# BosonHBC/BHRayTracer

Measured on AMD Instinct MI355X. Metric: Mrays/s (closest-hit + any-hit rays per second), with wall-clock per frame, higher is better.
Workload: dtype f32

## Files before the change

bhraytracer_amd/csrc/device_state.h:

```cpp
#pragma once

namespace bhrt {

template <class T> struct DevBuf {
    T *p = nullptr;
    size_t n = 0;
    DevBuf() = default;
    DevBuf(const DevBuf &) = delete;
    DevBuf &operator=(const DevBuf &) = delete;
    DevBuf(DevBuf &&o) noexcept : p(o.p), n(o.n) { o.p = nullptr; o.n = 0; }
    DevBuf &operator=(DevBuf &&o) noexcept
    {
        if (this != &o) { Free(); p = o.p; n = o.n; o.p = nullptr; o.n = 0; }
        return *this;
    }
    ~DevBuf() { Free(); }
    int Reserve(size_t want)
    {
        if (n >= want) return BHRT_OK;
        Free();
        HIP_CHECK(hipMalloc(&p, want * sizeof(T)));
        n = want;
        return BHRT_OK;
    }
// ... 115 lines not shown
    DevBuf<float> d_slowf;
    DevBuf<uint32_t> d_slowu;
    DevBuf<float> d_shf2;
    DevBuf<uint32_t> d_shu2;
    DevBuf<uint32_t> d_order_sh;
    DevBuf<uint32_t> d_seg_sh;
    DevBuf<Counters> d_cnt_sh;
    DevBuf<Counters> d_cnt;
    PinnedBuf<HostCounters> h_pub;
    HostCounters *d_pub = nullptr;
    uint32_t pub_seq = 0;
    int timers = 0;
    struct PendingTimer { int e0, e1; double *acc; };
    std::vector<PendingTimer> ev_pending;
    std::vector<int> ev_free;
    DevBuf<DPhoton> d_photons;
    uint32_t n_photons = 0;
    std::vector<HostPhoton> h_photons;
    DevBuf<float> d_ph_frames;
    DevBuf<float4> d_ph_hot, d_ph_cold, d_ph_dbox;
    PhotonMapDev pm;
    GatherWorkspace gw;
    struct Knobs {
        int stream_waves = -1;
        bool fused_camera = true;
        bool no_slow_queue = false;
        bool debug_slow = false, debug_gather = false, debug_drain = false;
        bool balance_host = false;
        int frame_cap = 0;
        int gather_lane_budget = 0;
        bool gather_counting_sort = false;
        bool shadow_overlap = true;
        bool fused_resolve = true;
        int gather_stats = 0;
        void FromEnv()
        {
            if (const char *e = getenv("BHRT_STREAM_WAVES")) stream_waves = atoi(e);
            if (const char *e = getenv("BHRT_FUSED_CAMERA")) fused_camera = atoi(e) != 0;
            no_slow_queue = getenv("BHRT_NO_SLOW_QUEUE") != nullptr;
            debug_slow = getenv("BHRT_DEBUG_SLOW") != nullptr; debug_gather = getenv("BHRT_DEBUG_GATHER") != nullptr; debug_drain = getenv("BHRT_DEBUG_DRAIN") != nullptr;
            if (const char *e = getenv("BHRT_PHOTON_BALANCE_HOST")) balance_host = atoi(e) != 0;
            if (const char *e = getenv("BHRT_GATHER_COUNTING_SORT")) gather_counting_sort = atoi(e) != 0;
            if (const char *e = getenv("BHRT_SHADOW_OVERLAP")) shadow_overlap = atoi(e) != 0;
            if (const char *e = getenv("BHRT_FUSED_RESOLVE")) fused_resolve = atoi(e) != 0;
        }
    } knobs;
    uint64_t pass_hint_key = 0;
    uint32_t pass_hint = 0;
    uint64_t frames_seen_key = 0;
    double frames_seen = 0;
    size_t frame_px = 0;
    DevBuf<uint8_t> d_frame_rgb;
    DevBuf<float> d_frame_rad, d_frame_var;
    DevBuf<uint32_t> d_frame_cnt;
    DevBuf<uint8_t> d_ad;
    DevBuf<uint8_t> d_dn;
    size_t api_cap = 0;
    DevBuf<float> d_api_f;
    DevBuf<int32_t> d_api_i;
};

void DestroyDeviceState(DeviceState *d)
{
    if (!d) return;
    if (d->device >= 0) (void)hipSetDevice(d->device);
    delete d;
}

}
```

bhraytracer_amd/csrc/kernels.hip:

```cpp
#include <hip/hip_runtime.h>

#include <stdlib.h>
#include <string.h>

#include <algorithm>
#include <type_traits>
#include <chrono>
#include <string>
#include <vector>

#include "bhrt.h"
#include "denoise.h"
#include "device_color24.h"
#include "device_photon.h"
#include "photon_host.h"
#include "scene_internal.h"

namespace bhrt {

#define HIP_CHECK(expr)                                                                                        \
    do {                                                                                                       \
        hipError_t e_ = (expr);                                                                                \
        if (e_ != hipSuccess) {                                                                                \
            SetError(std::string(#expr) + ": " + hipGetErrorString(e_));                                       \
// ... 184 lines not shown
{
    const uint32_t lane = __lane_id();
    const uint64_t lt = (1ull << lane) - 1ull;
    const uint64_t m0 = __ballot(cls == RC_HEAVY), m1 = __ballot(cls == RC_MEDIUM), m2 = __ballot(cls == RC_LIGHT), m3 = __ballot(cls == RC_MESH);
    uint32_t base = 0;
    if (lane < 4) {
        const uint64_t mk = lane == 0 ? m0 : (lane == 1 ? m1 : (lane == 2 ? m2 : m3));
        const uint32_t c = (uint32_t)__popcll(mk);
        if (c) base = atomicAdd(&cnt->cls[lane][shard].v, c);
    }
    const uint32_t wshard = shard;
    const uint32_t b0 = __shfl(base, 0), b1 = __shfl(base, 1), b2 = __shfl(base, 2), b3 = __shfl(base, 3);
    if (cls != RC_NONE) {
        const uint64_t mm = cls == RC_HEAVY ? m0 : (cls == RC_MEDIUM ? m1 : (cls == RC_LIGHT ? m2 : m3));
        const uint32_t pos = (cls == RC_HEAVY ? b0 : (cls == RC_MEDIUM ? b1 : (cls == RC_LIGHT ? b2 : b3))) + (uint32_t)__popcll(mm & lt);
        if (pos < ord.shard_cap) ord.idx[((size_t)cls * BHRT_ORDER_SHARDS + wshard) * ord.shard_cap + pos] = i;
        else atomicOr(&cnt->overflow.v, 8u);
    }
}
__device__ inline uint32_t shading_class(uint32_t meta, const Hit &hit)
{
    const uint32_t kind = meta & 15u;
    const bool is_hit = hit.node >= 0;
    bool heavy = false;
    if (is_hit) {
        if (kind == RK_CAMERA) heavy = true;
        else if (kind == RK_GI) heavy = fabsf(hit.t) > BHRT_BIAS;
        else if (kind == RK_REFR_IN) heavy = hit.front != 0;
        else heavy = true;
    }
    return heavy ? RC_HEAVY : ((kind == RK_REFR_IN && is_hit) ? RC_MEDIUM : RC_LIGHT);
}

struct SlowQueue {
    RayQueue q;
    uint32_t cap;
};
constexpr uint32_t kSlowCap = 1u << 16;
template <bool kPark, bool kCamera, bool kMeshes = true>
__global__ void __launch_bounds__(kBlock) k_trace_closest(DevScene S, PassInfo P, RayQueue q, uint32_t n, int uniform_side, HitBuf h, RayOrder ord, Counters *cnt,
                                                          SlowQueue slow )
{
    __shared__ bhrt_bvh_node nodelet[(kPark || !kMeshes) ? 1 : BHRT_LDS_NODES];
    const uint32_t i = blockIdx.x * blockDim.x + threadIdx.x;
    bool active = i < n;
    V3 o = v3(0, 0, 0), d = v3(0, 0, 1);
    uint32_t meta = 0;
    if (active) fetch_ray<kCamera>(S, P, q, i, o, d, meta);
    const bool has_meta = kCamera || q.meta;
    const int side = has_meta ? (int)((meta >> 4) & 3u) : uniform_side;
    const bool dead = has_meta && (meta & 15u) == RK_DEAD;
    Hit hit;
    uint32_t key = 0;
    bool is_slow = false;
    int parked = trace_closest<kMeshes>(S, o, d, side, hit, active && !dead, (kPark || !kMeshes) ? nullptr : nodelet, 0, kPark, kPark ? &key : nullptr,
                                        (uint16_t *)nullptr, 0, BHRT_LDS_NODES, kCamera, kPark ? &is_slow : nullptr);
    if (kPark && parked >= 0 && is_slow && slow.cap) {
        const uint32_t k = atomicAdd(&cnt->n_slow.v, 1u);
        if (k < slow.cap) {
            slow.q.ox[k] = o.x; slow.q.oy[k] = o.y; slow.q.oz[k] = o.z; slow.q.dx[k] = d.x; slow.q.dy[k] = d.y; slow.q.dz[k] = d.z;
            slow.q.frame[k] = kCamera ? i : q.frame[i];
            slow.q.meta[k] = meta;
            slow.q.rng_ctr[k] = (kCamera || (meta & 15u) == RK_GI) ? 0u : q.rng_ctr[i];
            active = false;
            parked = -1;
        }
    }
    if (active) { h.t[i] = hit.t; h.node[i] = hit.node; h.prim[i] = hit.prim; h.front[i] = hit.front | ((parked + 1) << 8); }
    if (kPark && parked >= 0) {
        ord.park_key[i] = key;
        if (!kCamera) ord.park_rank[i] = atomicAdd(&ord.park_bucket[key], 1u);
    }
    if (!ord.idx) return;
    uint32_t cls = RC_NONE;
    if (active && !dead) cls = parked >= 0 ? (uint32_t)RC_MESH : shading_class(meta, hit);
    file_ray(cls, i, (i >> 10) & (BHRT_ORDER_SHARDS - 1) , ord, cnt);
}
__device__ inline bool parked_entry(const RayOrder &ord, uint32_t b, uint32_t *s_seg, uint32_t &i, uint32_t first_entry = 0 )
{
    __syncthreads();
    if (threadIdx.x < 64) {
        const uint32_t l = threadIdx.x;
        const uint32_t a = l <= BHRT_ORDER_SHARDS ? ord.mesh_start[l] : 0xffffffffu;
        const uint32_t n_le = (uint32_t)__popcll(__ballot(l < BHRT_ORDER_SHARDS && a <= b));
        if (l == 0) *s_seg = n_le - 1;
    }
    __syncthreads();
    if (b >= ord.mesh_start[BHRT_ORDER_SHARDS]) return false;
    const uint32_t seg = *s_seg;
    const uint32_t local = (b - ord.mesh_start[seg]) * kBlock + first_entry + threadIdx.x;
    const bool active = local < ord.mesh_count[seg];
    i = active ? ord.idx[((size_t)RC_MESH * BHRT_ORDER_SHARDS + seg) * ord.shard_cap + local] : 0xffffffffu;
    return true;
}
#ifndef BHRT_XCD_LOCAL
#define BHRT_XCD_LOCAL 0
#endif
__device__ inline bool xcd_slice(uint32_t b, uint32_t nb, uint32_t &slice)
{
    slice = b;
#if BHRT_XCD_LOCAL
    constexpr uint32_t G = BHRT_XCD_LOCAL, span = 8 * G;
    const uint32_t chunk = b / span, in = b % span;
    if ((chunk + 1) * span <= nb) slice = chunk * span + (in & 7u) * G + (in >> 3);
#endif
    return b < nb;
}
__global__ void __launch_bounds__(kBlock) k_park_scatter(RayOrder ord)
{
    __shared__ uint32_t s_seg;
    uint32_t i;
    for (uint32_t b = blockIdx.x; parked_entry(ord, b, &s_seg, i); b += gridDim.x)
        if (i != 0xffffffffu) ord.park_sorted[ord.park_bucket[ord.park_key[i]] + ord.park_rank[i]] = i;
}
constexpr uint32_t kMeshNodelet = 256;
#ifndef BHRT_MESH_BLOCK
#define BHRT_MESH_BLOCK 64
#endif
constexpr int kMeshBlock = BHRT_MESH_BLOCK;
template <bool kCamera, int kPath, bool kLS = false>
__global__ void __launch_bounds__(kCamera ? kBlock : kMeshBlock, kPath == 1 ? 6 : 4 ) k_trace_mesh(DevScene S, PassInfo P, RayQueue q, HitBuf h, RayOrder ord, Counters *cnt)
{
    typedef typename std::conditional<kPath == 2, uint32_t, uint16_t>::type PathT;
    constexpr int kTB = kCamera ? kBlock : kMeshBlock;
    __shared__ bhrt_bvh_node nodelet[kPath ? 1 : kMeshNodelet];
    __shared__ PathT path[kPath ? 33 * kTB : 1];
    __shared__ uint32_t s_seg;
    bool active;
    uint32_t i;
    uint32_t slice;
    if (kCamera) {
        if (!xcd_slice(blockIdx.x, ord.mesh_start[BHRT_ORDER_SHARDS], slice)) return;
        if (!parked_entry(ord, slice, &s_seg, i)) return;
        active = i != 0xffffffffu;
        if (!active) i = 0;
    } else {
        const uint32_t total = ord.mesh_count[BHRT_ORDER_SHARDS];
        if (!xcd_slice(blockIdx.x, (total + kTB - 1) / kTB, slice)) return;
        const uint32_t k = slice * kTB + threadIdx.x;
        active = k < total;
        i = active ? ord.park_sorted[k] : 0u;
    }
    V3 o = v3(0, 0, 0), d = v3(0, 0, 1);
    uint32_t meta = 0;
    Hit hit = {BHRT_BIGFLOAT, -1, -1, 1};
    int start = 0;
    if (active) {
        fetch_ray<kCamera>(S, P, q, i, o, d, meta);
        hit.t = h.t[i]; hit.node = h.node[i]; hit.prim = h.prim[i];
        const int fw = h.front[i];
        hit.front = fw & 0xff;
        start = (fw >> 8) - 1;
    }
    trace_closest<true, PathT, kLS>(S, o, d, (int)((meta >> 4) & 3u), hit, active, kPath ? nullptr : nodelet, active ? start : S.n_nodes, false, nullptr,
                               kPath ? path + threadIdx.x : (PathT *)nullptr, kTB, kMeshNodelet);
    if (active) { h.t[i] = hit.t; h.node[i] = hit.node; h.prim[i] = hit.prim; h.front[i] = hit.front; }
    if (kCamera) file_ray(active ? shading_class(meta, hit) : (uint32_t)RC_NONE, i, slice & (BHRT_ORDER_SHARDS - 1), ord, cnt);
}
#ifndef BHRT_STREAM_REFILL
#define BHRT_STREAM_REFILL 32
#endif
constexpr int kStreamRefill = BHRT_STREAM_REFILL;
#ifndef BHRT_STREAM_OCC
#define BHRT_STREAM_OCC 6
#endif
#ifdef BHRT_DEBUG_DRAIN
__device__ unsigned long long g_stream_t[4];
#endif
#ifdef BHRT_DEBUG_STREAM
__device__ unsigned long long g_stream_dbg[8];
#endif
template <int kPath, bool kLS = false>
__global__ void __launch_bounds__(64, kPath == 1 ? BHRT_STREAM_OCC : (BHRT_STREAM_OCC < 5 ? BHRT_STREAM_OCC : 5) ) k_trace_mesh_stream(DevScene S, RayQueue q, HitBuf h, RayOrder ord, Counters *cnt)
{
    typedef typename std::conditional<kPath == 2, uint32_t, uint16_t>::type PathT;
    __shared__ PathT path[33 * 64];
    const uint32_t total = ord.mesh_count[BHRT_ORDER_SHARDS];
    const uint32_t lane = threadIdx.x;
    PathT *stack = path + lane;
    bool have = false, pending = false, exhausted = false;
    uint32_t i = 0;
    int n = 0, side = 0;
    Hit hit = {BHRT_BIGFLOAT, -1, -1, 1};
    MeshWalk W = {};
    W.st = 3;
    int cur_n = -1;
    MeshRef M = mesh_ref(S, 0);
#ifdef BHRT_DEBUG_STREAM
    unsigned long long dbg[8] = {0, 0, 0, 0, 0, 0, 0, 0};
    unsigned long long c_mark = __builtin_readcyclecounter();
// ... 69 lines not shown
#endif
        for (;;) {
            const int nD = __popcll(__ballot(W.st == 0)), nL = __popcll(__ballot(W.st == 1)), nC = __popcll(__ballot(W.st == 2));
            const int walking = nD + nL + nC;
            if (walking == 0 || (!exhausted && 64 - walking - n_wait >= kStreamRefill)) break;
#ifdef BHRT_DEBUG_STREAM
#if BHRT_FUSED_CLIMB
            dbg[0]++; dbg[1] += walking; dbg[2] += (nD >= nL && nD > 0) ? nD : nL;
            if (nD >= nL && nD > 0) dbg[6]++; else if (nL > 0) dbg[7]++;
#else
            dbg[0]++; dbg[1] += walking; dbg[2] += (nD >= nL && nD >= nC) ? nD : (nL >= nC ? nL : nC);
            if (nD >= nL && nD >= nC) dbg[6]++; else if (nL >= nC) dbg[7]++;
#endif
#endif
#ifdef BHRT_DEBUG_STREAM
            const unsigned long long r0 = __builtin_readcyclecounter();
#endif
            walk_round<PathT, kLS>(M, W, side, hit.t, hit.prim, hit.front, stack, 64u, nD, nL, nC);
#ifdef BHRT_DEBUG_STREAM
            if (nD >= nL && nD > 0) dbg[4] += __builtin_readcyclecounter() - r0;
#endif
        }
#ifdef BHRT_DEBUG_STREAM
        { const unsigned long long c = __builtin_readcyclecounter(); dbg[3] += c - c_mark; c_mark = c; }
#endif
    }
#ifdef BHRT_DEBUG_STREAM
    if (lane == 0) for (int k = 0; k < 8; k++) atomicAdd(&g_stream_dbg[k], dbg[k]);
#endif
#ifdef BHRT_DEBUG_DRAIN
    if (lane == 0) atomicMax(&g_stream_t[2], wall_clock64());
#endif
}
__global__ void __launch_bounds__(kBlock) k_file_parked(RayQueue q, HitBuf h, RayOrder ord, Counters *cnt)
{
    __shared__ uint32_t s_seg;
    uint32_t i;
    if (!parked_entry(ord, blockIdx.x, &s_seg, i)) return;
    const bool active = i != 0xffffffffu;
    uint32_t cls = RC_NONE;
    if (active) {
        Hit hit;
        hit.t = h.t[i]; hit.node = h.node[i]; hit.prim = h.prim[i]; hit.front = h.front[i];
        cls = shading_class(q.meta[i], hit);
    }
    file_ray(cls, active ? i : 0u, blockIdx.x & (BHRT_ORDER_SHARDS - 1), ord, cnt);
}

__global__ void __launch_bounds__(64) k_trace_slow(DevScene S, SlowQueue slow, uint32_t a, uint32_t b, HitBuf h)
{
    __shared__ CoopLds lds;
    __builtin_amdgcn_s_setprio(3);
    const uint32_t i = a + blockIdx.x;
    if (i >= b) return;
    const V3 o = v3(slow.q.ox[i], slow.q.oy[i], slow.q.oz[i]), d = v3(slow.q.dx[i], slow.q.dy[i], slow.q.dz[i]);
    const uint32_t meta = slow.q.meta[i];
    Hit hit;
#ifdef BHRT_DEBUG_LONG_RAYS
    const unsigned long long c0 = wall_clock64();
#endif
    trace_closest_coop(S, lds, o, d, (int)((meta >> 4) & 3u), hit);
#ifdef BHRT_DEBUG_LONG_RAYS
    const double ms = (double)(wall_clock64() - c0) / 1e5;
    if (threadIdx.x == 0 && ms > 5.0) printf("slow ray %u: %.1f ms o=(%.9g %.9g %.9g) d=(%.9g %.9g %.9g) side %u -> node %d prim %d t %.9g\n", i, ms, o.x, o.y, o.z, d.x, d.y, d.z, (meta >> 4) & 3u, hit.node, hit.prim, hit.t);
#endif
    if (threadIdx.x == 0) { h.t[i] = hit.t; h.node[i] = hit.node; h.prim[i] = hit.prim; h.front[i] = hit.front; }
}
__global__ void __launch_bounds__(kBlock) k_inject_slow(RayQueue sq, HitBuf sh, uint32_t src0, uint32_t m, RayQueue q, HitBuf h, uint32_t dst0)
{
    const uint32_t k = blockIdx.x * blockDim.x + threadIdx.x;
    if (k >= m) return;
    const uint32_t a = src0 + k, b = dst0 + k;
    q.ox[b] = sq.ox[a]; q.oy[b] = sq.oy[a]; q.oz[b] = sq.oz[a]; q.dx[b] = sq.dx[a]; q.dy[b] = sq.dy[a]; q.dz[b] = sq.dz[a];
    q.frame[b] = sq.frame[a]; q.meta[b] = sq.meta[a]; q.rng_ctr[b] = sq.rng_ctr[a];
    h.t[b] = sh.t[a]; h.node[b] = sh.node[a]; h.prim[b] = sh.prim[a]; h.front[b] = sh.front[a];
}
static inline uint32_t kFileAllBlocks(uint32_t first, uint32_t n) { return (n - (first & ~63u) + kBlock - 1) / kBlock; }
// ... 363 lines not shown
                code = pcode * 2;
                how = FH_REFR_FRONT;
            } else {
                code = pcode * 2;
                how = FH_REFR_OUT;
                const bhrt_material &pm = S.materials[(F.info[owner] >> 20) & 0xfffu];
                V3 af = v3(dm::powf_(BHRT_EULER, -pm.absorption[0] * hit.t), dm::powf_(BHRT_EULER, -pm.absorption[1] * hit.t),
                           dm::powf_(BHRT_EULER, -pm.absorption[2] * hit.t));
                mult = ld3i(F.refr_color, owner) * af;
            }
        }
        F.parent[f] = owner;
        F.info2[f] = (uint32_t)(gi + 64) | ((uint32_t)(bounce & 0xff) << 8);
        F.skey[f] = skey;
        F.code[f] = code;
        if (how == FH_REFR_OUT) st3(F.mult, f, mult);
        const int mi = kFm ? resolve_material(S, F.fm, hit.node, hit.prim) : S.nodes[hit.node].material;
        bool need_uv = kTex && mi >= 0 && (S.materials[mi].diffuse.map >= 0 || S.materials[mi].specular.map >= 0);
        if (kLe && mi >= 0) need_uv = need_uv || F.emission[mi].map >= 0;
        Attr a;
        hit_attrs(S, o, d, hit.t, hit.node, hit.prim, need_uv, a);
        shade_entry<kTex, kLe, kFm>(S, R, F, f, how, o, a, hit.node, mi, bounce, gi, code, skey, so);
        ray_owner = f;
    } else if (active) {
        if (kind == RK_CAMERA) {
            int pi, pj;
            uint32_t osmp;
            if (root_of) root_of[owner] = kNoRootFrame;
            else {
                slot_pixel(P, owner, pi, pj, osmp);
                st3(samples, sample_addr(P, owner), kTex ? tc_sample(S, S.background, v3((float)pi / S.cam.width, (float)pj / S.cam.height, 0.0f)) : ld3(S.background.color));
            }
        } else if (kind == RK_GI) {
            V3 mult = ld3i(F.gi_mult, owner);
            V3 outc = v3(0, 0, 0);
            if (is_hit) {
                outc = outc + v3(0, 0, 0) * mult;
            } else if (d.x == d.y && d.x == 0) {
                outc = outc + v3(1.0f, 0.0f, 1.0f);
            } else {
                V3 env = (kTex ? sample_environment(S, S.environment, d) : ld3(S.environment.color)) * mult;
                if (!(isnan_f(env.x) || isnan_f(env.y) || isnan_f(env.z))) outc = outc + env;
            }
            if (isnan_f(outc.x)) outc = v3(1.0f, 0.0f, 1.0f);
            else outc = clamp_white(outc);
            st3(F.gi, owner, outc);
        } else if (kind == RK_REFR_IN) {
            if (!is_hit) {
                st3(F.refr, owner, v3(1.0f, 0.0f, 1.0f));
            } else {
                Attr a;
                hit_attrs(S, o, d, hit.t, hit.node, hit.prim, false, a);
                const bhrt_material &m = S.materials[(F.info[owner] >> 20) & 0xfffu];
                const float refrGloss = m.glossiness > 50 ? m.glossiness : 0.f;
                V3 vN = a.N;
                V3 vV = -d;
                float cosPhi1 = dot(vV, -vN);
                float sinPhi1 = sqrtf(1 - cosPhi1 * cosPhi1);
                float sinPhi2 = m.ior * sinPhi1;
                if (sinPhi2 <= 1) {
                    float cosPhi2 = sqrtf(1 - sinPhi2 * sinPhi2);
                    V3 vTn = vN * cosPhi2;
                    V3 vNxV = cross(vN, vV);
                    V3 vTp = normalized(cross(vN, vNxV)) * sinPhi2;
                    V3 vT = vTn + vTp;
                    V3 vT_sampled = normalized(vT);
                    if (refrGloss > 0) {
                        DRng g;
                        g.key = bhrt_section_key(F.skey[owner], F.code[owner], BHRT_SEC_REFRACTION);
                        g.ctr = ctr;
                        float dotSign = 0;
                        int guard = 0;
                        while (dotSign <= 0 && guard++ < BHRT_MAXLOOP) {
                            float theta = 0;
                            vT_sampled = sample_along_light_direction(g, vT, refrGloss, theta);
                            dotSign = dot(vT_sampled, vN);
                        }
                        ctr = g.ctr;
                    }
                    so.has_refr = true;
                    so.rd = normalized(vT_sampled);
                    so.ro = a.p + vN * BHRT_BIAS;
                    so.rmeta = make_meta(RK_REFR_OUT, BHRT_HIT_FRONT, bounce);
                    so.rctr = ctr;
                } else if (bounce <= 0) {
                    st3(F.refr, owner, v3(0, 0, 0));
                } else {
                    V3 vR = ((-2 * cosPhi1) * vN - vV);
                    so.has_refr = true;
                    so.rd = vR;
                    so.ro = a.p - vN * BHRT_BIAS;
                    so.rmeta = make_meta(RK_REFR_IN, BHRT_HIT_FRONT_AND_BACK, bounce - 1);
                    so.rctr = ctr;
                }
            }
        } else {
            st3(F.refr, owner, clamp_white(ld3i(F.refr_color, owner) * (kTex ? sample_environment(S, S.environment, d) : ld3(S.environment.color))));
        }
    }

    uint32_t r0, r1, s0;
    block_alloc3(lds, &cnt->n_next.v, so.has_refr ? 1u : 0u, so.has_gi ? 1u : 0u, &cnt->n_shadow.v, so.has_shadow ? 1u : 0u, nullptr, 0u, r0, r1, s0, u2);
    if (so.has_refr) {
        if (r0 < R.cap_rays) put_ray(qout, r0, so.ro, so.rd, ray_owner, so.rmeta, so.rctr);
        else flag_overflow(cnt, 2u);
    }
    if (so.has_gi) {
        if (r1 < R.cap_rays) put_ray(qout, r1, so.go, so.gd, ray_owner, make_meta(RK_GI, BHRT_HIT_FRONT, 0), 0);
        else flag_overflow(cnt, 2u);
    }
    if (so.has_shadow) {
        if (s0 < R.cap_shadow) {
            qs.ox[s0] = so.so.x; qs.oy[s0] = so.so.y; qs.oz[s0] = so.so.z; qs.dx[s0] = so.sd.x; qs.dy[s0] = so.sd.y; qs.dz[s0] = so.sd.z;
            qs.tmax[s0] = so.stmax; qs.frame[s0] = ray_owner;
        } else flag_overflow(cnt, 4u);
    }
}
template <bool kCamera, bool kTex, bool kFused = false, bool kLe = false, bool kFm = false>
__global__ void __launch_bounds__(kShadeBlock, BHRT_SHADE_WAVES) k_shade(DevScene S, RenderParams R, PassInfo P, RayQueue qin, HitBuf hb, uint32_t n, RayQueue qout,
                                                   ShadowQueue qs, Frames F, float *samples, uint32_t *root_of, Counters *cnt, RayOrder ord, HostCounters *pub, uint32_t seq)
{
    shade_block<kCamera, kTex, kFused, kLe, kFm>(S, R, P, qin, hb, n, qout, qs, F, samples, root_of, cnt, ord);
    if (!pub) return;
    __syncthreads();
    if (threadIdx.x == 0 && atomicAdd(&cnt->shade_done.v, 1u) == gridDim.x - 1u) {
        __hip_atomic_store(&cnt->shade_done.v, 0u, __ATOMIC_RELAXED, __HIP_MEMORY_SCOPE_AGENT);
        publish_counters(cnt, pub, seq);
    }
}

template <bool kEmit>
// ... 1143 lines not shown
static decltype(&k_trace_mesh<true, 1>) MeshKernel(bool cam_step, int path_mode, bool ls)
{
    if (!cam_step) return path_mode == 1 ? k_trace_mesh<false, 1> : path_mode == 2 ? k_trace_mesh<false, 2> : k_trace_mesh<false, 0>;
    if (path_mode == 1) return ls ? k_trace_mesh<true, 1, true> : k_trace_mesh<true, 1>;
    if (path_mode == 2) return ls ? k_trace_mesh<true, 2, true> : k_trace_mesh<true, 2>;
    return k_trace_mesh<true, 0>;
}
static decltype(&k_trace_mesh_stream<1>) StreamKernel(int path_mode, bool ls)
{
    if (path_mode == 1) return ls ? k_trace_mesh_stream<1, true> : k_trace_mesh_stream<1>;
    return ls ? k_trace_mesh_stream<2, true> : k_trace_mesh_stream<2>;
}
static decltype(&k_shadow_mesh<1>) AnyHitMeshKernel(int path_mode, bool ls)
{
    if (path_mode == 1) return ls ? k_shadow_mesh<1, true> : k_shadow_mesh<1>;
    if (path_mode == 2) return ls ? k_shadow_mesh<2, true> : k_shadow_mesh<2>;
    return k_shadow_mesh<0>;
}
static decltype(&k_shade<true, true>) ShadeKernel(bool fused, bool cam_step, bool tex, bool le, bool fm)
{
    if (fm && !fused) {
        if (le && tex) return cam_step ? k_shade<true, true, false, true, true> : k_shade<false, true, false, true, true>;
        if (cam_step) return tex ? k_shade<true, true, false, false, true> : k_shade<true, false, false, false, true>;
        return tex ? k_shade<false, true, false, false, true> : k_shade<false, false, false, false, true>;
    }
    if (le && tex) {
        if (fused) return k_shade<true, true, true, true>;
        return cam_step ? k_shade<true, true, false, true> : k_shade<false, true, false, true>;
    }
    if (fused) return tex ? k_shade<true, true, true> : k_shade<true, false, true>;
    if (cam_step) return tex ? k_shade<true, true> : k_shade<true, false>;
    return tex ? k_shade<false, true> : k_shade<false, false>;
}
static decltype(&k_trace_closest<true, true>) ClosestKernel(bool park, bool cam_step, bool meshes)
{
    if (park) return cam_step ? k_trace_closest<true, true> : k_trace_closest<true, false>;
    if (!meshes) return cam_step ? k_trace_closest<false, true, false> : k_trace_closest<false, false, false>;
    return cam_step ? nullptr : k_trace_closest<false, false, true>;
}

#ifdef BHRT_DEBUG_DRAIN
static int DebugDrainReset()
{
    unsigned long long t0[4] = {~0ull, ~0ull, 0, 0};
    HIP_CHECK(hipMemcpyToSymbol(HIP_SYMBOL(g_stream_t), t0, sizeof(t0)));
    return BHRT_OK;
}
static int DebugDrainReport(DeviceState *D, uint32_t n_cur)
{
    unsigned long long t1[4];
    HIP_CHECK(hipMemcpyFromSymbol(t1, HIP_SYMBOL(g_stream_t), sizeof(t1)));
    static double dbg_total = 0, dbg_drain = 0;
    if (t1[1] != ~0ull) { dbg_total += (double)(t1[2] - t1[0]) / 1e5; dbg_drain += (double)(t1[2] - t1[1]) / 1e5; }
    if (D->knobs.debug_drain) fprintf(stderr, "mesh launch: %u rays, %.3f ms, of which %.3f ms after the list ran out (sums %.1f / %.1f ms)\n", n_cur, (double)(t1[2] - t1[0]) / 1e5, t1[1] != ~0ull ? (double)(t1[2] - t1[1]) / 1e5 : 0.0, dbg_total, dbg_drain);
    return BHRT_OK;
}
#else
static inline int DebugDrainReset() { return BHRT_OK; }
static inline int DebugDrainReport(DeviceState *, uint32_t) { return BHRT_OK; }
#endif
#ifdef BHRT_DEBUG_STREAM
static int DebugStreamReport()
{
    unsigned long long d[8], z[8] = {0, 0, 0, 0, 0, 0, 0, 0};
    HIP_CHECK(hipMemcpyFromSymbol(d, HIP_SYMBOL(g_stream_dbg), sizeof(d)));
    HIP_CHECK(hipMemcpyToSymbol(HIP_SYMBOL(g_stream_dbg), z, sizeof(z)));
    unsigned long long w[16], wz[16] = {};
    HIP_CHECK(hipMemcpyFromSymbol(w, HIP_SYMBOL(g_walk_dbg), sizeof(w)));
    HIP_CHECK(hipMemcpyToSymbol(HIP_SYMBOL(g_walk_dbg), wz, sizeof(wz)));
    fprintf(stderr, "walk: descend bodies %llu (%.1f lanes), exact boxes %llu (%.1f lanes), climbs %llu (%.1f lanes), climbs after a hit %llu (%.1f lanes), triangle slots %llu (%.1f lanes), barycentric parts %llu (%.1f lanes), exact grazing quotients %llu; exact boxes %llu; box-missed leaf siblings %llu, of them left out %llu\n",
            w[0], w[0] ? (double)w[1] / w[0] : 0., w[2], w[2] ? (double)w[3] / w[2] : 0., w[4], w[4] ? (double)w[5] / w[4] : 0., w[6], w[6] ? (double)w[7] / w[6] : 0., w[8],
            w[8] ? (double)w[9] / w[8] : 0., w[10], w[10] ? (double)w[11] / w[10] : 0., w[12], w[13], w[14], w[15]);
    fprintf(stderr, "stream: %llu rounds (%llu descend, %llu leaf), walking %.3f, in phase %.3f, clocks in rounds %.3g of which descend rounds %.3g, %llu refills\n", d[0], d[6],
            d[7], d[0] ? (double)d[1] / (64.0 * d[0]) : 0.0, d[0] ? (double)d[2] / (64.0 * d[0]) : 0.0, (double)d[3], (double)d[4], d[5]);
    return BHRT_OK;
}
#else
static inline int DebugStreamReport() { return BHRT_OK; }
#endif

#ifndef BHRT_INJECT_MIN_LOG2
#define BHRT_INJECT_MIN_LOG2 20
#endif
constexpr uint32_t kInjectMinRays = 1u << BHRT_INJECT_MIN_LOG2;

struct WavePass {
    typedef std::chrono::steady_clock::time_point TimePoint;
    DeviceState *const D;
    bhrt_stats *const st;
    const RenderParams &R;
    const PassInfo &P;
    const TimePoint wall0;
    const bool meshes, tex;
    const bool ls;
    const int path_mode;
    const uint32_t stream_waves;
    const bool sh_overlap;
    const bool lens;
    uint32_t *const root_of;
    const PassViews V;

    int cur = 0;
    uint32_t n_cur;
    bool first_step = true;
    bool injected = false;
    uint32_t n_extra = 0;
    uint32_t seq = 0;
    HostCounters hc = {};
    bool overflow = false;
    std::vector<uint32_t> frame_marks = {0};
    int sh_wait_par = 0; uint32_t sh_wait_n = 0;
    bool sh_pending[2] = {false, false};
    uint32_t slow_pending = 0, slow_traced = 0, slow_injected = 0;
    struct SlowBatch { uint32_t end; uint32_t step; hipEvent_t done; };
    std::vector<SlowBatch> slow_batches;
    size_t slow_batch_next = 0;
    uint64_t pass_closest = 0, pass_camera = 0, pass_shadow = 0, pass_deferred = 0;
    uint32_t pass_steps = 0;

    bool CamStep() const { return first_step && !lens; }
    bool Fused() const { return CamStep() && !meshes && D->knobs.fused_camera; }
    double MsSince(TimePoint t0) const { return std::chrono::duration<double>(std::chrono::steady_clock::now() - t0).count() * 1e3; }

    WavePass(bhrt_scene *scene, const bhrt_opts &o, bhrt_stats *stats, const RenderParams &Rp, const PassInfo &Pp, bool fuse_root, TimePoint render_start)
        : D(scene->dev), st(stats), R(Rp), P(Pp), wall0(render_start), meshes(scene->flat.hdr()->n_meshes > 0), tex(scene->flat.hdr()->n_texmaps > 0), ls(o.leaf_skip != 0),
          path_mode(PathMode(scene)), stream_waves(D->knobs.stream_waves >= 0 ? (uint32_t)D->knobs.stream_waves : D->n_cus * 4u * (uint32_t)BHRT_STREAM_OCC),
          sh_overlap(D->knobs.shadow_overlap && D->stream3 != nullptr && D->d_shf2.p != nullptr), lens(Pp.lens_r > 0.f), root_of(fuse_root ? D->d_root.p : nullptr),
          V(MakePassViews(D, sh_overlap)), n_cur(Pp.n_pixels * (uint32_t)Pp.spp)
    {
    }

    int Run()
    {
        BHRT_TRY(Begin());
        while (n_cur > 0 || slow_pending > slow_injected) {
            BHRT_TRY(MoveInSetAside());
            BHRT_TRY(TraceClosest());
            BHRT_TRY(Shade());
            if (!sh_overlap) LaunchAnyHit(D->stream, V.SQ, std::min<uint32_t>(n_cur + n_extra, R.cap_shadow), &D->d_cnt->n_shadow.v, V.RO, D->d_cnt);
            BHRT_TRY(ReadCounters());
            if (overflow) break;
            BHRT_TRY(TraceSetAside());
            if (sh_overlap) BHRT_TRY(QueueAnyHit());
            n_cur = hc.n_next;
            cur ^= 1;
            pass_steps++;
        }
        if (sh_overlap) for (int k = 0; k < 2; k++) if (sh_pending[k]) HIP_CHECK(hipStreamWaitEvent(D->stream, D->ev_shadow[k], 0));
        return BHRT_OK;
    }

    int Begin()
    {
        HIP_CHECK(hipMemsetAsync(D->d_cnt, 0, sizeof(Counters), D->stream));
        if (lens) {
            Timer t(D, &st->seconds_other);
            hipLaunchKernelGGL(k_lens_rays, dim3((n_cur + kBlock - 1) / kBlock), dim3(kBlock), 0, D->stream, D->S, P, V.Q[0], n_cur);
            t.Stop();
        }
        if (D->stream2) HIP_CHECK(hipStreamSynchronize(D->stream2));
        if (D->stream3) HIP_CHECK(hipStreamSynchronize(D->stream3));
// ... 15 lines not shown
            slow_injected = slow_pending;
            slow_batch_next = slow_batches.size();
            injected = true;
        } else if (!first_step && n_cur >= kInjectMinRays) {
            uint32_t upto = slow_injected;
            size_t b = slow_batch_next;
            while (b < slow_batches.size() && slow_batches[b].step + 2 <= pass_steps) { upto = slow_batches[b].end; b++; }
            if (upto > slow_injected && (uint64_t)n_cur + (upto - slow_injected) <= D->cap_rays) {
                HIP_CHECK(hipStreamWaitEvent(D->stream, slow_batches[b - 1].done, 0));
                n_extra = upto - slow_injected;
                hipLaunchKernelGGL(k_inject_slow, dim3((n_extra + kBlock - 1) / kBlock), dim3(kBlock), 0, D->stream, V.slowq.q, V.slow_hits, slow_injected, n_extra, V.Q[cur], V.HB, n_cur);
                if (D->knobs.debug_slow) fprintf(stderr, "slow rays: %u ride along with wave step %u (%u rays)\n", n_extra, pass_steps, n_cur);
                pass_deferred += n_extra;
                slow_injected = upto;
                slow_batch_next = b;
            }
        }
        return BHRT_OK;
    }

    int TraceClosest()
    {
        const RayOrder &RO = V.RO;
        const bool fused = Fused();
        if (fused) {
        } else if (injected) {
            Timer t(D, &st->seconds_trace_closest);
            hipLaunchKernelGGL(k_file_all, dim3((n_cur + kBlock - 1) / kBlock), dim3(kBlock), 0, D->stream, V.Q[cur], V.HB, 0u, n_cur, RO, D->d_cnt);
            t.Stop();
        } else {
            Timer t(D, &st->seconds_trace_closest);
            const SlowQueue no_slow = {V.slowq.q, 0u};
            if (meshes) BHRT_TRY(TraceThroughMeshes());
            else hipLaunchKernelGGL(ClosestKernel(false, CamStep(), false), dim3((n_cur + kBlock - 1) / kBlock), dim3(kBlock), 0, D->stream, D->S, P, V.Q[cur], n_cur, 0, V.HB, RO, D->d_cnt, no_slow);
            t.Stop();
        }
        if (n_extra) hipLaunchKernelGGL(k_file_all, dim3(kFileAllBlocks(n_cur, n_cur + n_extra)), dim3(kBlock), 0, D->stream, V.Q[cur], V.HB, n_cur, n_cur + n_extra, RO, D->d_cnt);
        if (!fused) {
            st->launches_trace_closest++;
            hipLaunchKernelGGL(k_order_prefix, dim3(1), dim3(128), 0, D->stream, D->d_cnt, RO);
        }
        return BHRT_OK;
    }

    int TraceThroughMeshes()
    {
        const RayOrder &RO = V.RO;
        const bool cam_step = CamStep();
        const dim3 tg((n_cur + kBlock - 1) / kBlock), tb(kBlock);
        const uint32_t n_buckets = 1u << BHRT_PARK_KEY_BITS;
        if (!cam_step) HIP_CHECK(hipMemsetAsync(RO.park_bucket, 0, n_buckets * sizeof(uint32_t), D->stream));
        hipLaunchKernelGGL(ClosestKernel(true, cam_step, true), tg, tb, 0, D->stream, D->S, P, V.Q[cur], n_cur, 0, V.HB, RO, D->d_cnt, V.slowq);
        hipLaunchKernelGGL(k_mesh_prefix, dim3(1), dim3(64), 0, D->stream, D->d_cnt, RO);
        if (!cam_step) {
            const dim3 pg(std::min<uint32_t>(tg.x + BHRT_ORDER_SHARDS, 4096u));
            LaunchExclusiveScan(D->stream, RO.park_bucket, n_buckets, RO.park_bucket + n_buckets);
            hipLaunchKernelGGL(k_park_scatter, pg, tb, 0, D->stream, RO);
        }
        if (sh_wait_n) {
            HIP_CHECK(hipEventRecord(D->ev_shade, D->stream));
            BHRT_TRY(LaunchQueuedAnyHit(D->ev_shade));
        }
        if (!cam_step && path_mode != 0 && stream_waves > 0) {
            BHRT_TRY(DebugDrainReset());
            hipLaunchKernelGGL(StreamKernel(path_mode, ls), dim3(std::min<uint32_t>((n_cur + 63) / 64, stream_waves)), dim3(64), 0, D->stream, D->S, V.Q[cur], V.HB, RO, D->d_cnt);
            BHRT_TRY(DebugDrainReport(D, n_cur));
        } else
            hipLaunchKernelGGL(MeshKernel(cam_step, path_mode, ls), cam_step ? dim3(tg.x + BHRT_ORDER_SHARDS)  : dim3((n_cur + kMeshBlock - 1) / kMeshBlock),
                               cam_step ? tb : dim3(kMeshBlock), 0, D->stream, D->S, P, V.Q[cur], V.HB, RO, D->d_cnt);
        if (!cam_step) hipLaunchKernelGGL(k_file_parked, dim3(tg.x + BHRT_ORDER_SHARDS), tb, 0, D->stream, V.Q[cur], V.HB, RO, D->d_cnt);
        return BHRT_OK;
    }

    int Shade()
    {
        const bool fused = Fused();
        seq = ++D->pub_seq;
        Timer t(D, &st->seconds_shade, 0);
        const dim3 sg((n_cur + n_extra + kShadeBlock - 1) / kShadeBlock + (fused ? 0 : 3 * BHRT_ORDER_SHARDS)), sb(kShadeBlock);
        const int par = (int)(pass_steps & 1u);
        if (sh_wait_n) { HIP_CHECK(hipEventRecord(D->ev_shade, D->stream)); BHRT_TRY(LaunchQueuedAnyHit(D->ev_shade)); }
        if (sh_overlap && sh_pending[par]) { HIP_CHECK(hipStreamWaitEvent(D->stream, D->ev_shadow[par], 0)); sh_pending[par] = false; }
        hipLaunchKernelGGL(ShadeKernel(fused, CamStep(), tex, V.F.le != nullptr, V.F.fm.tab != nullptr), sg, sb, 0, D->stream, D->S, R, P, V.Q[cur], V.HB, n_cur + n_extra, V.Q[cur ^ 1], (sh_overlap && par) ? V.SQ2 : V.SQ, V.F, D->d_samples, root_of, D->d_cnt, V.RO, D->d_pub, seq);
        t.Stop();
        if (sh_overlap) HIP_CHECK(hipEventRecord(D->ev_shade, D->stream));
        return BHRT_OK;
    }

    void LaunchAnyHit(hipStream_t stream, const ShadowQueue &sq, uint32_t n, const uint32_t *n_dev, const RayOrder &order, Counters *counters)
    {
        Timer t(D, &st->seconds_trace_shadow, 1, stream);
        const dim3 hg((n + kBlock - 1) / kBlock), hb(kBlock);
        if (meshes) {
            hipLaunchKernelGGL(k_trace_shadow_park, hg, hb, 0, stream, D->S, sq, n, n_dev, V.F.vis, order, counters);
            hipLaunchKernelGGL(k_mesh_prefix, dim3(1), dim3(64), 0, stream, counters, order);
            hipLaunchKernelGGL(AnyHitMeshKernel(path_mode, ls), dim3((hg.x + BHRT_ORDER_SHARDS) * (kBlock / kShadowBlock)), dim3(kShadowBlock), 0, stream, D->S, sq, V.F.vis, order);
        } else hipLaunchKernelGGL(k_trace_shadow<false>, hg, hb, 0, stream, D->S, sq, n, n_dev, V.F.vis);
        t.Stop();
    }

    int LaunchQueuedAnyHit(hipEvent_t after)
    {
        if (!sh_wait_n) return BHRT_OK;
// ... 276 lines not shown
        if (variance) HIP_CHECK(hipMemcpyAsync(variance, d_variance, npix * 12, hipMemcpyDeviceToHost, s));
        if (count) HIP_CHECK(hipMemcpyAsync(count, d_count, npix * 4, hipMemcpyDeviceToHost, s));
        HIP_CHECK(hipStreamSynchronize(s));
        return BHRT_OK;
    }
};

}

using namespace bhrt;

extern "C" {

int bhrt_device_count(int *n)
try {
    if (!n) { SetError("null argument"); return BHRT_ERR_ARG; }
    int c = 0;
    hipError_t e = hipGetDeviceCount(&c);
    if (e != hipSuccess) { *n = 0; SetError(std::string("hipGetDeviceCount: ") + hipGetErrorString(e)); return BHRT_ERR_NO_DEVICE; }
    *n = c;
    return BHRT_OK;
} catch (...) { return bhrt::AbiException(); }

int bhrt_scene_knob(bhrt_scene *scene, const char *name, int value)
try {
    int rc = EnsureUploaded(scene);
    if (rc) return rc;
    if (!name || value < 0) { SetError("knob: bad arguments"); return BHRT_ERR_ARG; }
    if (!strcmp(name, "frame_cap")) scene->dev->knobs.frame_cap = value;
    else if (!strcmp(name, "gather_lane_budget")) scene->dev->knobs.gather_lane_budget = value;
    else if (!strcmp(name, "gather_stats")) scene->dev->knobs.gather_stats = value;
    else if (!strcmp(name, "shadow_overlap")) scene->dev->knobs.shadow_overlap = value != 0;
    else if (!strcmp(name, "fused_resolve")) scene->dev->knobs.fused_resolve = value != 0;
    else { SetError(std::string("knob: unknown name ") + name); return BHRT_ERR_ARG; }
    return BHRT_OK;
} catch (...) { return bhrt::AbiException(); }

int bhrt_scene_upload(bhrt_scene *scene, int device)
try {
    if (!scene) { SetError("null scene"); return BHRT_ERR_ARG; }
    if (scene->dev && scene->dev->device == device) { HIP_CHECK(hipSetDevice(device)); return BHRT_OK; }
    int count = 0;
    if (hipGetDeviceCount(&count) != hipSuccess || count <= 0) { SetError("no HIP device available (this path has no CPU fallback)"); return BHRT_ERR_NO_DEVICE; }
    if (device < 0 || device >= count) { SetError("device index out of range"); return BHRT_ERR_ARG; }
    if (scene->max_bvh_depth > 64) { SetError("BVH deeper than 64 levels: the stackless trail holds 64"); return BHRT_ERR_UNSUPPORTED; }
    if (scene->dev) { DestroyDeviceState(scene->dev); scene->dev = nullptr; }
    HIP_CHECK(hipSetDevice(device));
    DeviceState *D = new DeviceState;
    D->knobs.FromEnv();
    D->device = device;
    scene->dev = D;
    {
        int cus = 0;
        if (hipDeviceGetAttribute(&cus, hipDeviceAttributeMultiprocessorCount, device) == hipSuccess && cus > 0) D->n_cus = (uint32_t)cus;
    }
    const std::vector<uint8_t> &blob = scene->flat.blob;
    const bhrt_flat_header *H = scene->flat.hdr();
    HIP_CHECK(hipStreamCreate(&D->stream));
    HIP_CHECK(hipEventCreate(&D->ev[0]));
    HIP_CHECK(hipEventCreate(&D->ev[1]));
    BHRT_TRY(D->d_blob.Reserve(blob.size()));
    HIP_CHECK(hipMemcpy(D->d_blob, blob.data(), blob.size(), hipMemcpyHostToDevice));
    std::vector<int32_t> chain((size_t)std::max<uint32_t>(H->n_nodes, 1) * BHRT_MAX_NODE_DEPTH, 0);
    const bhrt_node *nodes = (const bhrt_node *)(blob.data() + H->off_nodes);
    for (uint32_t n = 0; n < H->n_nodes; n++) {
        int k = nodes[n].depth - 1, c = (int)n;
// ... 70 lines not shown
    for (int i = 1; i < 32; i++) {
        auto halton = [](int index, int base) { float r = 0, f = 1.0f / (float)base; for (int k = index; k > 0; k /= base) { r += f * (k % base); f /= (float)base; } return r; };
        float x = halton(i, 2), y = halton(i, 3);
        float r = sqrtf(x) * 0.5f;
        S.tapx[i] = r * dm::sinf_(y * (float)M_PI * 2);
        S.tapy[i] = r * dm::cosf_(y * (float)M_PI * 2);
        if (!(fabsf(S.tapx[i]) <= 0.5f && fabsf(S.tapy[i]) <= 0.5f)) { SetError("footprint tap outside the half-unit disc"); return BHRT_ERR_UNSUPPORTED; }
    }
    return BHRT_OK;
} catch (...) { return bhrt::AbiException(); }

static int EnsureApiScratch(DeviceState *D, size_t n)
{
    if (D->api_cap >= n) return BHRT_OK;
    D->api_cap = 0;
    BHRT_TRY(D->d_api_f.Reserve(n * 9));
    BHRT_TRY(D->d_api_i.Reserve(n * 3));
    D->api_cap = n;
    return BHRT_OK;
}

int bhrt_trace_closest_dev(bhrt_scene *scene, const float *d_rays_soa, int hit_side, size_t n, bhrt_hits d_out, void *stream)
try {
    int rc = EnsureUploaded(scene);
    if (rc) return rc;
    if (!d_rays_soa || !d_out.t || !d_out.node || !d_out.prim || !d_out.front) { SetError("null buffer"); return BHRT_ERR_ARG; }
    if (hit_side < 1 || hit_side > 3) { SetError("hit_side must be 1, 2 or 3"); return BHRT_ERR_ARG; }
    if (n == 0) return BHRT_OK;
    if (n > 0x7fffffffu) { SetError("too many rays for one call"); return BHRT_ERR_ARG; }
    RayQueue q = MakeRayQueue(const_cast<float *>(d_rays_soa), nullptr, n);
    HitBuf h; h.t = d_out.t; h.node = d_out.node; h.prim = d_out.prim; h.front = d_out.front;
    hipStream_t s = stream ? (hipStream_t)stream : scene->dev->stream;
    RayOrder no_order = {nullptr, 0, nullptr, nullptr, nullptr, nullptr, nullptr, nullptr, nullptr, nullptr};
    auto closest_kernel = ClosestKernel(false, false, scene->flat.hdr()->n_meshes > 0);
    hipLaunchKernelGGL(closest_kernel, dim3((unsigned)((n + kBlock - 1) / kBlock)), dim3(kBlock), 0, s,
                       scene->dev->S, PassInfo(), q, (uint32_t)n, hit_side, h, no_order, (Counters *)nullptr, SlowQueue{q, 0u});
    HIP_CHECK(hipGetLastError());
    if (!stream) HIP_CHECK(hipStreamSynchronize(s));
    return BHRT_OK;
} catch (...) { return bhrt::AbiException(); }

int bhrt_trace_closest_host(bhrt_scene *scene, const float *rays_soa, int hit_side, size_t n, bhrt_hits out)
try {
    int rc = EnsureUploaded(scene);
    if (rc) return rc;
    if (n == 0) return BHRT_OK;
    if (!rays_soa || !out.t || !out.node || !out.prim || !out.front) { SetError("null buffer"); return BHRT_ERR_ARG; }
    DeviceState *D = scene->dev;
    rc = EnsureApiScratch(D, n);
    if (rc) return rc;
    HIP_CHECK(hipMemcpy(D->d_api_f, rays_soa, n * 6 * sizeof(float), hipMemcpyHostToDevice));
    bhrt_hits d; d.t = D->d_api_f + 6 * n; d.node = D->d_api_i; d.prim = D->d_api_i + n; d.front = D->d_api_i + 2 * n;
    rc = bhrt_trace_closest_dev(scene, D->d_api_f, hit_side, n, d, nullptr);
    if (rc) return rc;
    HIP_CHECK(hipMemcpy(out.t, d.t, n * sizeof(float), hipMemcpyDeviceToHost));
    HIP_CHECK(hipMemcpy(out.node, d.node, n * sizeof(int32_t), hipMemcpyDeviceToHost));
    HIP_CHECK(hipMemcpy(out.prim, d.prim, n * sizeof(int32_t), hipMemcpyDeviceToHost));
    HIP_CHECK(hipMemcpy(out.front, d.front, n * sizeof(int32_t), hipMemcpyDeviceToHost));
    return BHRT_OK;
} catch (...) { return bhrt::AbiException(); }

int bhrt_trace_shadow_dev(bhrt_scene *scene, const float *d_rays_soa, const float *d_tmax, size_t n, float *d_vis, void *stream)
try {
    int rc = EnsureUploaded(scene);
    if (rc) return rc;
    if (!d_rays_soa || !d_tmax || !d_vis) { SetError("null buffer"); return BHRT_ERR_ARG; }
    if (n == 0) return BHRT_OK;
    if (n > 0x7fffffffu) { SetError("too many rays for one call"); return BHRT_ERR_ARG; }
    ShadowQueue q = MakeShadowQueue(const_cast<float *>(d_rays_soa), nullptr, n);
// ... 791 lines not shown
```

Before: 6764.

## Resolve miss rays inside trace kernels instead of filing them for shading

Adds a MissSink so camera rays that miss are marked with no root frame directly in the trace kernels. With the knob at 2 or higher, GI and refraction-out misses also get their environment contribution computed there. Such rays are filed as RC_NONE, so the shading pass skips them and their hit records are never written. This cuts hit-buffer traffic and shading work for misses, at the cost of extra code, more template instantiations and environment sampling inside the trace kernel. By default (miss_in_trace=1) only the camera-miss early-out is active, because the GI and refraction sink pointers are left null.

```diff
diff --git a/bhraytracer_amd/csrc/device_state.h b/bhraytracer_amd/csrc/device_state.h
--- a/bhraytracer_amd/csrc/device_state.h
+++ b/bhraytracer_amd/csrc/device_state.h
@@ -171,6 +171,7 @@
         bool gather_counting_sort = false;
         bool shadow_overlap = true;
         bool fused_resolve = true;
+        int miss_in_trace = 1;
         int gather_stats = 0;
         void FromEnv()
         {
@@ -182,6 +183,7 @@
             if (const char *e = getenv("BHRT_GATHER_COUNTING_SORT")) gather_counting_sort = atoi(e) != 0;
             if (const char *e = getenv("BHRT_SHADOW_OVERLAP")) shadow_overlap = atoi(e) != 0;
             if (const char *e = getenv("BHRT_FUSED_RESOLVE")) fused_resolve = atoi(e) != 0;
+            if (const char *e = getenv("BHRT_MISS_IN_TRACE")) miss_in_trace = atoi(e);
         }
     } knobs;
     uint64_t pass_hint_key = 0;
diff --git a/bhraytracer_amd/csrc/kernels.hip b/bhraytracer_amd/csrc/kernels.hip
--- a/bhraytracer_amd/csrc/kernels.hip
+++ b/bhraytracer_amd/csrc/kernels.hip
@@ -240,14 +240,46 @@
     return heavy ? RC_HEAVY : ((kind == RK_REFR_IN && is_hit) ? RC_MEDIUM : RC_LIGHT);
 }
 
+struct MissSink {
+    const float *gi_mult, *refr_color;
+    float *gi, *refr;
+    uint32_t *root_of;
+};
+template <bool kTex>
+__device__ __forceinline__ void finish_miss(const DevScene &S, const MissSink &M, uint32_t kind, uint32_t owner, V3 d)
+{
+    if (kind == RK_GI) {
+        V3 mult = ld3i(M.gi_mult, owner);
+        V3 outc = v3(0, 0, 0);
+        if (d.x == d.y && d.x == 0) {
+            outc = outc + v3(1.0f, 0.0f, 1.0f);
+        } else {
+            V3 env = (kTex ? sample_environment(S, S.environment, d) : ld3(S.environment.color)) * mult;
+            if (!(isnan_f(env.x) || isnan_f(env.y) || isnan_f(env.z))) outc = outc + env;
+        }
+        if (isnan_f(outc.x)) outc = v3(1.0f, 0.0f, 1.0f);
+        else outc = clamp_white(outc);
+        st3(M.gi, owner, outc);
+    } else {
+        st3(M.refr, owner, clamp_white(ld3i(M.refr_color, owner) * (kTex ? sample_environment(S, S.environment, d) : ld3(S.environment.color))));
+    }
+}
+__device__ inline bool miss_ends_in_trace(const MissSink &M, uint32_t kind) { return ((kind == RK_GI || kind == RK_REFR_OUT) && M.gi) || (kind == RK_CAMERA && M.root_of); }
+template <bool kTex>
+__device__ __forceinline__ void end_miss(const DevScene &S, const MissSink &M, uint32_t kind, uint32_t owner, V3 d)
+{
+    if (kind == RK_CAMERA) M.root_of[owner] = kNoRootFrame;
+    else finish_miss<kTex>(S, M, kind, owner, d);
+}
+
 struct SlowQueue {
     RayQueue q;
     uint32_t cap;
 };
 constexpr uint32_t kSlowCap = 1u << 16;
-template <bool kPark, bool kCamera, bool kMeshes = true>
+template <bool kPark, bool kCamera, bool kMeshes = true, int kMiss = 0>
 __global__ void __launch_bounds__(kBlock) k_trace_closest(DevScene S, PassInfo P, RayQueue q, uint32_t n, int uniform_side, HitBuf h, RayOrder ord, Counters *cnt,
-                                                          SlowQueue slow )
+                                                          SlowQueue slow , MissSink miss )
 {
     __shared__ bhrt_bvh_node nodelet[(kPark || !kMeshes) ? 1 : BHRT_LDS_NODES];
     const uint32_t i = blockIdx.x * blockDim.x + threadIdx.x;
@@ -274,14 +306,19 @@
             parked = -1;
         }
     }
-    if (active) { h.t[i] = hit.t; h.node[i] = hit.node; h.prim[i] = hit.prim; h.front[i] = hit.front | ((parked + 1) << 8); }
+    bool ended = false;
+    if (kMiss != 0 && active && !dead && parked < 0 && hit.node < 0 && miss_ends_in_trace(miss, meta & 15u)) {
+        end_miss<kMiss == 2>(S, miss, meta & 15u, kCamera ? i : q.frame[i], d);
+        ended = true;
+    }
+    if (active && !ended) { h.t[i] = hit.t; h.node[i] = hit.node; h.prim[i] = hit.prim; h.front[i] = hit.front | ((parked + 1) << 8); }
     if (kPark && parked >= 0) {
         ord.park_key[i] = key;
         if (!kCamera) ord.park_rank[i] = atomicAdd(&ord.park_bucket[key], 1u);
     }
     if (!ord.idx) return;
     uint32_t cls = RC_NONE;
-    if (active && !dead) cls = parked >= 0 ? (uint32_t)RC_MESH : shading_class(meta, hit);
+    if (active && !dead && !ended) cls = parked >= 0 ? (uint32_t)RC_MESH : shading_class(meta, hit);
     file_ray(cls, i, (i >> 10) & (BHRT_ORDER_SHARDS - 1) , ord, cnt);
 }
 __device__ inline bool parked_entry(const RayOrder &ord, uint32_t b, uint32_t *s_seg, uint32_t &i, uint32_t first_entry = 0 )
@@ -327,7 +364,8 @@
 #endif
 constexpr int kMeshBlock = BHRT_MESH_BLOCK;
 template <bool kCamera, int kPath, bool kLS = false>
-__global__ void __launch_bounds__(kCamera ? kBlock : kMeshBlock, kPath == 1 ? 6 : 4 ) k_trace_mesh(DevScene S, PassInfo P, RayQueue q, HitBuf h, RayOrder ord, Counters *cnt)
+__global__ void __launch_bounds__(kCamera ? kBlock : kMeshBlock, kPath == 1 ? 6 : 4 ) k_trace_mesh(DevScene S, PassInfo P, RayQueue q, HitBuf h, RayOrder ord, Counters *cnt,
+                                                                                                                                                  uint32_t *root_of )
 {
     typedef typename std::conditional<kPath == 2, uint32_t, uint16_t>::type PathT;
     constexpr int kTB = kCamera ? kBlock : kMeshBlock;
@@ -362,8 +400,10 @@
     }
     trace_closest<true, PathT, kLS>(S, o, d, (int)((meta >> 4) & 3u), hit, active, kPath ? nullptr : nodelet, active ? start : S.n_nodes, false, nullptr,
                                kPath ? path + threadIdx.x : (PathT *)nullptr, kTB, kMeshNodelet);
-    if (active) { h.t[i] = hit.t; h.node[i] = hit.node; h.prim[i] = hit.prim; h.front[i] = hit.front; }
-    if (kCamera) file_ray(active ? shading_class(meta, hit) : (uint32_t)RC_NONE, i, slice & (BHRT_ORDER_SHARDS - 1), ord, cnt);
+    const bool ended = kCamera && root_of && active && hit.node < 0 && (meta & 15u) == RK_CAMERA;
+    if (ended) root_of[i] = kNoRootFrame;
+    if (active && !ended) { h.t[i] = hit.t; h.node[i] = hit.node; h.prim[i] = hit.prim; h.front[i] = hit.front; }
+    if (kCamera) file_ray(active && !ended ? shading_class(meta, hit) : (uint32_t)RC_NONE, i, slice & (BHRT_ORDER_SHARDS - 1), ord, cnt);
 }
 #ifndef BHRT_STREAM_REFILL
 #define BHRT_STREAM_REFILL 32
@@ -499,7 +539,8 @@
     if (lane == 0) atomicMax(&g_stream_t[2], wall_clock64());
 #endif
 }
-__global__ void __launch_bounds__(kBlock) k_file_parked(RayQueue q, HitBuf h, RayOrder ord, Counters *cnt)
+template <int kMiss>
+__global__ void __launch_bounds__(kBlock) k_file_parked(DevScene S, RayQueue q, HitBuf h, RayOrder ord, Counters *cnt, MissSink miss )
 {
     __shared__ uint32_t s_seg;
     uint32_t i;
@@ -509,7 +550,12 @@
     if (active) {
         Hit hit;
         hit.t = h.t[i]; hit.node = h.node[i]; hit.prim = h.prim[i]; hit.front = h.front[i];
-        cls = shading_class(q.meta[i], hit);
+        const uint32_t meta = q.meta[i];
+        cls = shading_class(meta, hit);
+        if (kMiss != 0 && hit.node < 0 && miss_ends_in_trace(miss, meta & 15u)) {
+            end_miss<kMiss == 2>(S, miss, meta & 15u, q.frame[i], v3(q.dx[i], q.dy[i], q.dz[i]));
+            cls = RC_NONE;
+        }
     }
     file_ray(cls, active ? i : 0u, blockIdx.x & (BHRT_ORDER_SHARDS - 1), ord, cnt);
 }
@@ -939,19 +985,14 @@
                 st3(samples, sample_addr(P, owner), kTex ? tc_sample(S, S.background, v3((float)pi / S.cam.width, (float)pj / S.cam.height, 0.0f)) : ld3(S.background.color));
             }
         } else if (kind == RK_GI) {
-            V3 mult = ld3i(F.gi_mult, owner);
-            V3 outc = v3(0, 0, 0);
             if (is_hit) {
+                V3 mult = ld3i(F.gi_mult, owner);
+                V3 outc = v3(0, 0, 0);
                 outc = outc + v3(0, 0, 0) * mult;
-            } else if (d.x == d.y && d.x == 0) {
-                outc = outc + v3(1.0f, 0.0f, 1.0f);
-            } else {
-                V3 env = (kTex ? sample_environment(S, S.environment, d) : ld3(S.environment.color)) * mult;
-                if (!(isnan_f(env.x) || isnan_f(env.y) || isnan_f(env.z))) outc = outc + env;
-            }
-            if (isnan_f(outc.x)) outc = v3(1.0f, 0.0f, 1.0f);
-            else outc = clamp_white(outc);
-            st3(F.gi, owner, outc);
+                if (isnan_f(outc.x)) outc = v3(1.0f, 0.0f, 1.0f);
+                else outc = clamp_white(outc);
+                st3(F.gi, owner, outc);
+            } else finish_miss<kTex>(S, MissSink{F.gi_mult, F.refr_color, F.gi, F.refr, nullptr}, RK_GI, owner, d);
         } else if (kind == RK_REFR_IN) {
             if (!is_hit) {
                 st3(F.refr, owner, v3(1.0f, 0.0f, 1.0f));
@@ -1001,9 +1042,7 @@
                     so.rctr = ctr;
                 }
             }
-        } else {
-            st3(F.refr, owner, clamp_white(ld3i(F.refr_color, owner) * (kTex ? sample_environment(S, S.environment, d) : ld3(S.environment.color))));
-        }
+        } else finish_miss<kTex>(S, MissSink{F.gi_mult, F.refr_color, F.gi, F.refr, nullptr}, RK_REFR_OUT, owner, d);
     }
 
     uint32_t r0, r1, s0;
@@ -2213,12 +2252,20 @@
     if (cam_step) return tex ? k_shade<true, true> : k_shade<true, false>;
     return tex ? k_shade<false, true> : k_shade<false, false>;
 }
-static decltype(&k_trace_closest<true, true>) ClosestKernel(bool park, bool cam_step, bool meshes)
-{
+static decltype(&k_trace_closest<true, true>) ClosestKernel(bool park, bool cam_step, bool meshes, int miss)
+{
+    if (miss == 1) {
+        if (park) return cam_step ? k_trace_closest<true, true, true, 1> : k_trace_closest<true, false, true, 1>;
+        if (!meshes) return cam_step ? k_trace_closest<false, true, false, 1> : k_trace_closest<false, false, false, 1>;
+    } else if (miss == 2) {
+        if (park) return cam_step ? k_trace_closest<true, true, true, 2> : k_trace_closest<true, false, true, 2>;
+        if (!meshes) return cam_step ? k_trace_closest<false, true, false, 2> : k_trace_closest<false, false, false, 2>;
+    }
     if (park) return cam_step ? k_trace_closest<true, true> : k_trace_closest<true, false>;
     if (!meshes) return cam_step ? k_trace_closest<false, true, false> : k_trace_closest<false, false, false>;
     return cam_step ? nullptr : k_trace_closest<false, false, true>;
 }
+static decltype(&k_file_parked<0>) FileParkedKernel(int miss) { return miss == 1 ? k_file_parked<1> : miss == 2 ? k_file_parked<2> : k_file_parked<0>; }
 
 #ifdef BHRT_DEBUG_DRAIN
 static int DebugDrainReset()
@@ -2280,6 +2327,8 @@
     const bool lens;
     uint32_t *const root_of;
     const PassViews V;
+    const int miss;
+    const MissSink sink;
 
     int cur = 0;
     uint32_t n_cur;
@@ -2307,7 +2356,8 @@
         : D(scene->dev), st(stats), R(Rp), P(Pp), wall0(render_start), meshes(scene->flat.hdr()->n_meshes > 0), tex(scene->flat.hdr()->n_texmaps > 0), ls(o.leaf_skip != 0),
           path_mode(PathMode(scene)), stream_waves(D->knobs.stream_waves >= 0 ? (uint32_t)D->knobs.stream_waves : D->n_cus * 4u * (uint32_t)BHRT_STREAM_OCC),
           sh_overlap(D->knobs.shadow_overlap && D->stream3 != nullptr && D->d_shf2.p != nullptr), lens(Pp.lens_r > 0.f), root_of(fuse_root ? D->d_root.p : nullptr),
-          V(MakePassViews(D, sh_overlap)), n_cur(Pp.n_pixels * (uint32_t)Pp.spp)
+          V(MakePassViews(D, sh_overlap)), miss(D->knobs.miss_in_trace <= 0 ? 0 : (scene->flat.hdr()->environment.map >= 0 ? 2 : 1)),
+          sink{V.F.gi_mult, V.F.refr_color, D->knobs.miss_in_trace >= 2 ? V.F.gi : nullptr, D->knobs.miss_in_trace >= 2 ? V.F.refr : nullptr, root_of}, n_cur(Pp.n_pixels * (uint32_t)Pp.spp)
     {
     }
 
@@ -2389,7 +2439,7 @@
             Timer t(D, &st->seconds_trace_closest);
             const SlowQueue no_slow = {V.slowq.q, 0u};
             if (meshes) BHRT_TRY(TraceThroughMeshes());
-            else hipLaunchKernelGGL(ClosestKernel(false, CamStep(), false), dim3((n_cur + kBlock - 1) / kBlock), dim3(kBlock), 0, D->stream, D->S, P, V.Q[cur], n_cur, 0, V.HB, RO, D->d_cnt, no_slow);
+            else hipLaunchKernelGGL(ClosestKernel(false, CamStep(), false, miss), dim3((n_cur + kBlock - 1) / kBlock), dim3(kBlock), 0, D->stream, D->S, P, V.Q[cur], n_cur, 0, V.HB, RO, D->d_cnt, no_slow, sink);
             t.Stop();
         }
         if (n_extra) hipLaunchKernelGGL(k_file_all, dim3(kFileAllBlocks(n_cur, n_cur + n_extra)), dim3(kBlock), 0, D->stream, V.Q[cur], V.HB, n_cur, n_cur + n_extra, RO, D->d_cnt);
@@ -2407,7 +2457,7 @@
         const dim3 tg((n_cur + kBlock - 1) / kBlock), tb(kBlock);
         const uint32_t n_buckets = 1u << BHRT_PARK_KEY_BITS;
         if (!cam_step) HIP_CHECK(hipMemsetAsync(RO.park_bucket, 0, n_buckets * sizeof(uint32_t), D->stream));
-        hipLaunchKernelGGL(ClosestKernel(true, cam_step, true), tg, tb, 0, D->stream, D->S, P, V.Q[cur], n_cur, 0, V.HB, RO, D->d_cnt, V.slowq);
+        hipLaunchKernelGGL(ClosestKernel(true, cam_step, true, miss), tg, tb, 0, D->stream, D->S, P, V.Q[cur], n_cur, 0, V.HB, RO, D->d_cnt, V.slowq, sink);
         hipLaunchKernelGGL(k_mesh_prefix, dim3(1), dim3(64), 0, D->stream, D->d_cnt, RO);
         if (!cam_step) {
             const dim3 pg(std::min<uint32_t>(tg.x + BHRT_ORDER_SHARDS, 4096u));
@@ -2424,8 +2474,8 @@
             BHRT_TRY(DebugDrainReport(D, n_cur));
         } else
             hipLaunchKernelGGL(MeshKernel(cam_step, path_mode, ls), cam_step ? dim3(tg.x + BHRT_ORDER_SHARDS)  : dim3((n_cur + kMeshBlock - 1) / kMeshBlock),
-                               cam_step ? tb : dim3(kMeshBlock), 0, D->stream, D->S, P, V.Q[cur], V.HB, RO, D->d_cnt);
-        if (!cam_step) hipLaunchKernelGGL(k_file_parked, dim3(tg.x + BHRT_ORDER_SHARDS), tb, 0, D->stream, V.Q[cur], V.HB, RO, D->d_cnt);
+                               cam_step ? tb : dim3(kMeshBlock), 0, D->stream, D->S, P, V.Q[cur], V.HB, RO, D->d_cnt, miss ? root_of : (uint32_t *)nullptr);
+        if (!cam_step) hipLaunchKernelGGL(FileParkedKernel(miss), dim3(tg.x + BHRT_ORDER_SHARDS), tb, 0, D->stream, D->S, V.Q[cur], V.HB, RO, D->d_cnt, sink);
         return BHRT_OK;
     }
 
@@ -2768,6 +2818,7 @@
     else if (!strcmp(name, "gather_stats")) scene->dev->knobs.gather_stats = value;
     else if (!strcmp(name, "shadow_overlap")) scene->dev->knobs.shadow_overlap = value != 0;
     else if (!strcmp(name, "fused_resolve")) scene->dev->knobs.fused_resolve = value != 0;
+    else if (!strcmp(name, "miss_in_trace")) scene->dev->knobs.miss_in_trace = value;
     else { SetError(std::string("knob: unknown name ") + name); return BHRT_ERR_ARG; }
     return BHRT_OK;
 } catch (...) { return bhrt::AbiException(); }
@@ -2904,9 +2955,9 @@
     HitBuf h; h.t = d_out.t; h.node = d_out.node; h.prim = d_out.prim; h.front = d_out.front;
     hipStream_t s = stream ? (hipStream_t)stream : scene->dev->stream;
     RayOrder no_order = {nullptr, 0, nullptr, nullptr, nullptr, nullptr, nullptr, nullptr, nullptr, nullptr};
-    auto closest_kernel = ClosestKernel(false, false, scene->flat.hdr()->n_meshes > 0);
+    auto closest_kernel = ClosestKernel(false, false, scene->flat.hdr()->n_meshes > 0, 0);
     hipLaunchKernelGGL(closest_kernel, dim3((unsigned)((n + kBlock - 1) / kBlock)), dim3(kBlock), 0, s,
-                       scene->dev->S, PassInfo(), q, (uint32_t)n, hit_side, h, no_order, (Counters *)nullptr, SlowQueue{q, 0u});
+                       scene->dev->S, PassInfo(), q, (uint32_t)n, hit_side, h, no_order, (Counters *)nullptr, SlowQueue{q, 0u}, MissSink{nullptr, nullptr, nullptr, nullptr, nullptr});
     HIP_CHECK(hipGetLastError());
     if (!stream) HIP_CHECK(hipStreamSynchronize(s));
     return BHRT_OK;
```

Result: no change. 6760 (median of 2 runs) (-0.1%).
